# mohammed-amr/detectInBlur

Measured on AMD Instinct MI355X. Metric: blurred imgs/sec @800x1333 (--gpu_blur sparse correlation, fp16, batch 8), higher is better.
Workload: dtype f16; 1 GPU; configs[1]: --gpu_blur batch=8 3x800x1333 fp16, param_index=1 (expl 0.005), low_exposure fractions {1/18,1/10,1/5}, bit-exact accumulation; batch_per_gpu=8, parallelism=image-parallel x1

## Files before the change

### detectinblur_amd/csrc/dib_blur.hip

```cpp
#include "dib_compact_dev.h"
#include <mutex>
#include <stdlib.h>
#include <string.h>

extern "C" { __device__ __attribute__((used)) unsigned *dib_status_word = nullptr; }
#define DIB_STATUS_HANDOFF 1u
#define DIB_STATUS_GEOMETRY 2u
#define DIB_STATUS_WORDS 16
#ifdef DIB_STEP_POLLSTATS
extern "C" { __device__ __attribute__((used)) unsigned dib_poll_stats[4] = {0, 0, 0, 0}; }
#endif

namespace dib {

__device__ __forceinline__ void report_and_exit(unsigned code, unsigned detail) {
  typedef __attribute__((address_space(1))) unsigned gu32;
  gu32 *st = (gu32 *)(size_t)*(unsigned *volatile *)&dib_status_word;
  __hip_atomic_store(st + 1, detail, __ATOMIC_RELAXED, __HIP_MEMORY_SCOPE_SYSTEM);
  __hip_atomic_store(st, code, __ATOMIC_RELAXED, __HIP_MEMORY_SCOPE_SYSTEM);
  __builtin_amdgcn_endpgm();
}

typedef _Float16 h2 __attribute__((ext_vector_type(2)));
typedef unsigned uvec2 __attribute__((ext_vector_type(2)));
// ... 647 lines not shown
      for (int k = 0; k < NK; ++k) {
        bool z;
        coff[k] = 2u * (unsigned)map_coord_sel(c_first + lane + 32 * k, W, pa, pb, mode, z);
        zmask |= z ? 1u << k : 0u;
      }
    }
    if (!zero_mode && r_first >= 0 && r_first + LROWS - 1 <= H - 1) {
      const int s0 = (r_first + qb) * w2;
#pragma unroll
      for (int g = 0; g < GQ; ++g) soff[g] = s0 + g * w2;
    } else {
      const int nrows = TH + (w.rl - w.rf);
#pragma unroll
      for (int g = 0; g < GQ; ++g) {
        bool zr;
        const int sr = map_coord_sel(r_first + min(qb + g, nrows - 1), H, pa, pb, mode, zr);
        zmask |= zr ? 1u << (8 + g) : 0u;
        soff[g] = sr * w2;
      }
    }
    const bool masked = __builtin_amdgcn_ballot_w64(zmask != 0) != 0;
#pragma unroll
    for (int part = 0; part < PARTS; ++part) {
#pragma unroll
      for (int g = 0; g < GP; ++g) {
        if (part * GP + g >= GQ) continue;
        const int so = __builtin_amdgcn_readfirstlane(soff[part * GP + g]);
#pragma unroll
        for (int k = 0; k < NK; ++k) v[g][k] = __builtin_amdgcn_raw_buffer_load_b16(in_rsrc, coff[k], so, 0);
      }
      DIB_TL_STAMP(sg == 0 && part == 0, 40);
      if (part == 0 && sg > 0) __syncthreads();
      const int wl = fresh_lane();
      const unsigned wp = lds0 + (unsigned)((qb + part * GP) * QPITCH + wl * 8);
      if constexpr (L) {
#pragma unroll
        for (int g = 0; g < GP; ++g) {
          if (part * GP + g >= GQ) continue;
          unsigned u[NK];
#pragma unroll
          for (int k = 0; k < NK; ++k)
            u[k] = (masked && (((zmask >> k) & 1u) || ((zmask >> (8 + part * GP + g)) & 1u))) ? 0u : (unsigned)(unsigned short)v[g][k];
          uvec2 e;
          e.x = u[0] | (u[1] << 16);
          e.y = u[2] | (u[3] << 16);
          *(lds_u2 *)(size_t)(wp + (unsigned)(g * QPITCH)) = e;
          if (wl < 32) {
            uvec2 f;
            f.x = u[2] | (u[3] << 16);
            f.y = u[4] | (u[5] << 16);
            *(lds_u2 *)(size_t)(wp + (unsigned)(g * QPITCH + 512)) = f;
          }
        }
      } else if (wl < QUAD_PITCH) {
        if (!masked) {
#pragma unroll
          for (int g = 0; g < GP; ++g) {
            if (part * GP + g >= GQ) continue;
            uvec2 e;
            typedef short s2v __attribute__((ext_vector_type(2)));
            e.x = __builtin_bit_cast(unsigned, s2v{v[g][0], v[g][1]});
            e.y = __builtin_bit_cast(unsigned, s2v{v[g][2], v[g][3]});
            *(lds_u2 *)(size_t)(wp + (unsigned)(g * QPITCH)) = e;
          }
        } else {
#pragma unroll
          for (int g = 0; g < GP; ++g) {
            if (part * GP + g >= GQ) continue;
            unsigned u[4];
#pragma unroll
            for (int k = 0; k < 4; ++k)
              u[k] = (((zmask >> k) & 1u) || ((zmask >> (8 + part * GP + g)) & 1u)) ? 0u : (unsigned)(unsigned short)v[g][k];
            uvec2 e;
            e.x = u[0] | (u[1] << 16);
            e.y = u[2] | (u[3] << 16);
            *(lds_u2 *)(size_t)(wp + (unsigned)(g * QPITCH)) = e;
          }
        }
      }
    }
    __syncthreads();
    DIB_TL_STAMP(sg == 0, 16);
    if constexpr (STEP) { if (sg == 0 && (nsegs >> 30)) wait_tables(); }
    const int tl = fresh_lane();
    const unsigned lane_addr = lds0 + (unsigned)((wave * 8 + (tl >> 5) * 4) * QPITCH + (tl & 31) * 8);
    if constexpr (ACC == DIB_ACC_FP32) {
      if (W - x0f() <= 64) tap_loop_quad_fp32<true, L>(acc32, ltaps, w.t0, w.n, lane_addr);
      else tap_loop_quad_fp32<false, L>(acc32, ltaps, w.t0, w.n, lane_addr);
    } else if constexpr (ACC == DIB_ACC_FAST16) {
      const unsigned long long vg = uniform64((unsigned long long)(tab + table_vgroups_off(K)));
      if (!use_vruns) {
        if (W - x0f() <= 64) tap_loop_quad<true, true, L>(acc, ltaps, w.t0, w.n, lane_addr);
        else tap_loop_quad<true, false, L>(acc, ltaps, w.t0, w.n, lane_addr);
      } else if (W - x0f() <= 64) tap_loop_quad_vrun<true>(acc, vg, w.t0, lane_addr);
      else tap_loop_quad_vrun<false>(acc, vg, w.t0, lane_addr);
    } else {
      if (W - x0f() <= 64) tap_loop_quad<ACC == DIB_ACC_FMA16, true, L>(acc, ltaps, w.t0, w.n, lane_addr);
      else tap_loop_quad<ACC == DIB_ACC_FMA16, false, L>(acc, ltaps, w.t0, w.n, lane_addr);
    }
  }
  if constexpr (ACC == DIB_ACC_FP32) {
#pragma unroll
    for (int i = 0; i < 8; ++i) acc[i] = h2{(_Float16)acc32[2 * i], (_Float16)acc32[2 * i + 1]};
  }
  DIB_TL_STAMP(true, 24);
#undef DIB_TL_STAMP
  if constexpr (NORM) {
    const int Hp = na->Hp, Wp = na->Wp, nhwc = na->nhwc;
    const float m = na->mean[img][ch], sd = na->std[img][ch];
    const unsigned long long a = uniform64((unsigned long long)d.out + (nhwc ? (unsigned long long)ch * 4ull : (unsigned long long)ch * Hp * Wp * 4ull));
    const __amdgpu_buffer_rsrc_t out_rsrc = __builtin_amdgcn_make_buffer_rsrc((void *)a, 0, Hp * Wp * 4 * (nhwc ? 3 : 1) - (nhwc ? ch * 4 : 0), 0x00020000);
    const int x0 = x0f(), y0 = y0f();
    const int sl = fresh_lane();
    const int yl = y0 + wave * 8 + (sl >> 5) * 4, xl = x0 + (sl & 31);
    const unsigned px = nhwc ? 12u : 4u;
    const unsigned base = (unsigned)(yl * Wp + xl) * px, oob = 0x7ffffff0u;
    const bool inside = x0 + QTILE_W <= W && y0 + TH <= H;
#pragma unroll
    for (int i = 0; i < 4; ++i) {
      const unsigned ro = base + (unsigned)(i * Wp) * px;
      const float v[4] = {(float)acc[2 * i].x, (float)acc[2 * i].y, (float)acc[2 * i + 1].x, (float)acc[2 * i + 1].y};
#pragma unroll
      for (int q = 0; q < 4; ++q) {
        const int col = xl + 32 * q, row = yl + i;
        const bool in_img = inside || (row < H && col < W);
        const float f = in_img ? (v[q] - m) / sd : 0.f;
        __builtin_amdgcn_raw_buffer_store_b32(__builtin_bit_cast(int, f), out_rsrc, (in_img || (row < Hp && col < Wp)) ? ro + 32u * q * px : oob, 0, 0);
      }
    }
  } else {
    int chs = ch;
    if constexpr (STEP) asm volatile("" : "+s"(chs));
    const __amdgpu_buffer_rsrc_t out_rsrc = plane_rsrc(d.out, chs, H, W);
    const int x0 = x0f(), y0 = y0f();
    const int sl = fresh_lane();
    const int yl = y0 + wave * 8 + (sl >> 5) * 4, xl = x0 + (sl & 31);
    const unsigned base = (unsigned)(yl * w2 + xl * 2), oob = 0x7ffffff0u;
    if (x0 + QTILE_W <= W && y0 + TH <= H) {
      typedef int i4v __attribute__((ext_vector_type(4)));
      const unsigned long long pa2 = uniform64((unsigned long long)d.out + (unsigned long long)chs * H * W * 2ull);
      const i4v rs = {(int)(unsigned)pa2, (int)(unsigned)(pa2 >> 32) & 0xffff, H * W * 2, 0x00020000};
      int so = 0;
#pragma unroll
      for (int i = 0; i < 4; ++i) {
        asm volatile("buffer_store_short %0, %2, %3, %4 offen\n\t"
                     "buffer_store_short_d16_hi %0, %2, %3, %4 offen offset:64\n\t"
                     "buffer_store_short %1, %2, %3, %4 offen offset:128\n\t"
                     "buffer_store_short_d16_hi %1, %2, %3, %4 offen offset:192"
                     :: "v"(acc[2 * i]), "v"(acc[2 * i + 1]), "v"(base), "s"(rs), "s"(so) : "memory");
        so += w2;
      }
      return;
    }
#pragma unroll
    for (int i = 0; i < 4; ++i) {
      const bool row_ok = yl + i < H;
      const unsigned a0 = __builtin_bit_cast(unsigned, acc[2 * i]), a1 = __builtin_bit_cast(unsigned, acc[2 * i + 1]);
      const unsigned ro = base + (unsigned)(i * w2);
      __builtin_amdgcn_raw_buffer_store_b16((short)(a0 & 0xffffu), out_rsrc, row_ok && xl < W ? ro : oob, 0, 0);
      __builtin_amdgcn_raw_buffer_store_b16((short)(a0 >> 16), out_rsrc, row_ok && xl + 32 < W ? ro + 64u : oob, 0, 0);
      __builtin_amdgcn_raw_buffer_store_b16((short)(a1 & 0xffffu), out_rsrc, row_ok && xl + 64 < W ? ro + 128u : oob, 0, 0);
      __builtin_amdgcn_raw_buffer_store_b16((short)(a1 >> 16), out_rsrc, row_ok && xl + 96 < W ? ro + 192u : oob, 0, 0);
    }
  }
}

#ifdef DIB_TIMELINE
__device__ unsigned long long *g_timeline;
#define DIB_TL_SLOT (*(unsigned long long *volatile *)&g_timeline)
constexpr int TL_WORD = QLDS_BYTES / 4;
#endif

template <int ACC, int KC, bool FLAT = false>
__global__ __launch_bounds__(256, 8) void blur_quad_f16_kernel(BlurBatch batch, FlatBands fb) {
  constexpr int K = KC;
  extern __shared__ unsigned nlds[];
  int img_i = blockIdx.y, entry = blockIdx.x >> 3;
  if constexpr (FLAT) {
    typedef int i16v __attribute__((ext_vector_type(16)));
    const i16v bb = *reinterpret_cast<const i16v *>(fb.begin[blockIdx.x & 7]);
    const int len = bb[15];
// ... 50 lines not shown
  unsigned lds_words;
  __device__ __forceinline__ void operator()() const {
    static_assert(STEP_REPLICA_WORDS * 4 == 128, "the shift below");
#ifdef DIB_PORTABLE_TAPS
    {
      const uvec2 sp = lds_b64(lds_words), tb = lds_b64(lds_words + 8);
      const unsigned xcc = __builtin_amdgcn_s_getreg((2 << 11) | 20);
      const unsigned *ctr = reinterpret_cast<const unsigned *>((((unsigned long long)(unsigned)__builtin_amdgcn_readfirstlane((int)sp.y) << 32) |
                                                                 (unsigned)__builtin_amdgcn_readfirstlane((int)sp.x)) + 128ull * xcc);
      const unsigned target = (unsigned)__builtin_amdgcn_readfirstlane((int)tb.x), budget = (unsigned)__builtin_amdgcn_readfirstlane((int)tb.y);
      for (unsigned spins = 0;; ++spins) {
        if ((int)(__hip_atomic_load(ctr, __ATOMIC_RELAXED, __HIP_MEMORY_SCOPE_AGENT) - target) >= 0) return;
        if (spins >= budget) report_and_exit(DIB_STATUS_HANDOFF, target);
        __builtin_amdgcn_s_sleep(2);
      }
    }
#endif
    asm volatile(
        "v_mov_b32 v48, %0\n\t"
        "ds_read_b64 v[46:47], v48\n\t"
        "ds_read_b64 v[44:45], v48 offset:8\n\t"
        "s_getreg_b32 s39, hwreg(20, 0, 3)\n\t"
        "s_lshl_b32 s39, s39, 7\n\t"
        "s_waitcnt lgkmcnt(0)\n\t"
        "v_readfirstlane_b32 s36, v46\n\t"
        "v_readfirstlane_b32 s37, v47\n\t"
        "v_readfirstlane_b32 s38, v44\n\t"
        "s_add_u32 s36, s36, s39\n\t"
        "s_addc_u32 s37, s37, 0\n\t"
        "v_readfirstlane_b32 s39, v45\n\t"
        "s_load_dword s40, s[36:37], 0x0\n\t"
        "s_mov_b32 s41, 0\n\t"
        "s_waitcnt lgkmcnt(0)\n\t"
        "s_sub_u32 s40, s40, s38\n\t"
        "s_cmp_lt_i32 s40, 0\n\t"
        "s_cbranch_scc0 Ldibw_done%=\n\t"
        "v_mov_b32 v48, 0\n\t"
        "Ldibw_poll%=:\n\t"
        "global_load_dword v48, v48, s[36:37] sc1\n\t"
        "s_waitcnt vmcnt(0)\n\t"
        "v_readfirstlane_b32 s40, v48\n\t"
        "v_mov_b32 v48, 0\n\t"
        "s_sub_u32 s40, s40, s38\n\t"
        "s_cmp_lt_i32 s40, 0\n\t"
        "s_cbranch_scc0 Ldibw_done%=\n\t"
        "s_sleep 2\n\t"
        "s_add_u32 s41, s41, 1\n\t"
        "s_cmp_lt_u32 s41, s39\n\t"
        "s_cbranch_scc1 Ldibw_poll%=\n\t"
        "s_getpc_b64 s[36:37]\n\t"
        "s_add_u32 s36, s36, dib_status_word@rel32@lo+4\n\t"
        "s_addc_u32 s37, s37, dib_status_word@rel32@hi+12\n\t"
        "s_load_dwordx2 s[36:37], s[36:37], 0x0\n\t"
        "v_mov_b32 v47, s38\n\t"
        "v_mov_b32 v46, 1\n\t"
        "s_waitcnt lgkmcnt(0)\n\t"
        "global_store_dword v48, v47, s[36:37] offset:4 sc0 sc1\n\t"
        "global_store_dword v48, v46, s[36:37] sc0 sc1\n\t"
        "s_waitcnt vmcnt(0)\n\t"
        "s_endpgm\n\t"
        "Ldibw_done%=:\n\t"
#ifdef DIB_STEP_POLLSTATS
        "s_cmp_lt_u32 s41, 33\n\t"
        "s_cbranch_scc1 Ldibw_nostat%=\n\t"
        "s_getpc_b64 s[36:37]\n\t"
        "s_add_u32 s36, s36, dib_poll_stats@rel32@lo+4\n\t"
        "s_addc_u32 s37, s37, dib_poll_stats@rel32@hi+12\n\t"
        "v_mov_b32 v48, 0\n\t"
        "global_load_dword v47, v48, s[36:37] offset:4 sc1\n\t"
        "s_waitcnt vmcnt(0)\n\t"
        "v_readfirstlane_b32 s40, v47\n\t"
        "s_cmp_le_u32 s41, s40\n\t"
        "s_cbranch_scc1 Ldibw_nostat%=\n\t"
        "v_mov_b32 v47, s41\n\t"
        "global_atomic_umax v48, v47, s[36:37] offset:4\n\t"
        "Ldibw_nostat%=:\n\t"
#endif
        :: "s"(lds_words)
        : "s36", "s37", "s38", "s39", "s40", "s41", "v44", "v45", "v46", "v47", "v48", "scc", "memory");
  }
};
static_assert(DIB_STATUS_HANDOFF == 1u, "the v_mov_b32 v46, 1 above");

template <int ACC>
__global__ __launch_bounds__(256, 8) void blur_step_f16_kernel(BlurBatch batch, StepSync sy, PsfPtrs psfs) {
  constexpr int K = 128;
  extern __shared__ unsigned nlds[];
  const ImageDesc d = batch.img[blockIdx.y];
  asm volatile("" ::"s"(d.in), "s"(d.out), "s"(d.C), "s"(d.H), "s"(d.W), "s"(d.table), "s"(d.tiles_x), "s"(d.tiles_y),
               "s"(d.inv_per_ch), "s"(d.inv_tiles_x), "s"(d.tab), "s"(sy.sync), "s"(sy.target), "s"(sy.ncx), "s"(sy.row), "s"(sy.rec));
  const int wave = __builtin_amdgcn_readfirstlane((int)threadIdx.x >> 6);
  if (blockIdx.x < (unsigned)sy.ncx) {
    if (blockIdx.y == 0 && blockIdx.x < (unsigned)sy.n_psf && !(sy.flags & COMPACT_DEBUG_NOSIGNAL)) {
      unsigned *rec = sy.rec + (size_t)blockIdx.x * (STEP_REPLICAS * STEP_REC_WORDS);
#ifdef DIB_STEP_STAMPS
      unsigned long long *dbg = *(unsigned long long *volatile *)&g_step_stamps;
      if (dbg) dbg += 8 * blockIdx.x;
      compact_psf_f16_wg256<true, true>(psfs.p[blockIdx.x], sy.flags, sy.tables + (size_t)blockIdx.x * table_words(K), (lds_u32 *)nlds, wave, rec, sy.target, dbg);
#else
      compact_psf_f16_wg256<true, true>(psfs.p[blockIdx.x], sy.flags, sy.tables + (size_t)blockIdx.x * table_words(K), (lds_u32 *)nlds, wave, rec, sy.target);
#endif
      asm volatile("s_waitcnt vmcnt(0)" ::: "memory");
      __syncthreads();
      const int t = wave * 64 + (int)__builtin_amdgcn_mbcnt_hi(~0u, __builtin_amdgcn_mbcnt_lo(~0u, 0u));
#ifdef DIB_STEP_STAMPS
      if (dbg && t == 0) dbg[6] = __builtin_amdgcn_s_memrealtime();
#endif
      if (t < STEP_REPLICAS)
        __hip_atomic_fetch_add(sy.sync + t * STEP_REPLICA_WORDS, 1u, __ATOMIC_RELAXED, __HIP_MEMORY_SCOPE_AGENT);
#ifdef DIB_STEP_STAMPS
      asm volatile("s_waitcnt vmcnt(0)" ::: "memory");
      if (dbg && t == 0) dbg[7] = __builtin_amdgcn_s_memrealtime();
#endif
    }
    return;
  }
  const unsigned bx = blockIdx.x - (unsigned)sy.ncx;
  const int per_ch = d.tiles_x * d.tiles_y;
  int local;
  if (!band_entry(d.C * per_ch, bx & 7, bx >> 3, local)) __builtin_amdgcn_endpgm();
#ifdef DIB_STEP_STAMPS
  unsigned long long *bdbg = *(unsigned long long *volatile *)&g_step_stamps;
  if (bdbg && blockIdx.y == 0 && wave == 0) { bdbg += 8 * MAX_BATCH + 4 * bx; bdbg[0] = __builtin_amdgcn_s_memrealtime(); } else bdbg = nullptr;
#endif
  int early = 1;
  if (blockIdx.y * (unsigned)sy.row + blockIdx.x >= STEP_EARLY) {
    unsigned c;
    asm volatile("s_load_dword %0, %1, 0x0\n\ts_waitcnt lgkmcnt(0)" : "=s"(c) : "s"(sy.sync + (blockIdx.x & 7) * STEP_REPLICA_WORDS) : "memory");
    early = (int)((c - sy.target) >> 31);
  }
  asm volatile("" : "+s"(early));
  int nsegs0 = 0;
  uint4 seg0 = make_uint4(0, 0, 0, 0);
  if (early) {
    const unsigned long long *pr = reinterpret_cast<const unsigned long long *>(sy.rec + ((size_t)d.table * STEP_REPLICAS + (blockIdx.x & (STEP_REPLICAS - 1))) * STEP_REC_WORDS);
#ifdef DIB_STEP_POLLSTATS
    unsigned pspins = 0;
#endif
    for (unsigned spins = 0;; ++spins) {
#ifdef DIB_STEP_POLLSTATS
      pspins = spins;
#endif
      const unsigned long long ra = __hip_atomic_load(pr, __ATOMIC_RELAXED, __HIP_MEMORY_SCOPE_AGENT);
      const unsigned long long rb = __hip_atomic_load(pr + 1, __ATOMIC_RELAXED, __HIP_MEMORY_SCOPE_AGENT);
      const unsigned ta = __builtin_amdgcn_readfirstlane((unsigned)(ra >> 32)), tb = __builtin_amdgcn_readfirstlane((unsigned)(rb >> 32));
      if (ta == sy.target && tb == sy.target) {
        const unsigned a = __builtin_amdgcn_readfirstlane((unsigned)ra), b2 = __builtin_amdgcn_readfirstlane((unsigned)rb);
        nsegs0 = (int)(a >> 16);
        seg0 = make_uint4(0u, a & 0xffffu, b2 >> 16, b2 & 0xffffu);
        break;
      }
      if (spins > sy.poll_budget) report_and_exit(DIB_STATUS_HANDOFF, sy.target);
      __builtin_amdgcn_s_sleep(2);
    }
#ifdef DIB_STEP_POLLSTATS
    if (pspins > 32 && wave == 0 && __builtin_amdgcn_mbcnt_hi(~0u, __builtin_amdgcn_mbcnt_lo(~0u, 0u)) == 0 &&
        pspins > __hip_atomic_load(&dib_poll_stats[0], __ATOMIC_RELAXED, __HIP_MEMORY_SCOPE_AGENT))
      atomicMax(&dib_poll_stats[0], pspins);
#endif
    if (__builtin_amdgcn_mbcnt_hi(~0u, __builtin_amdgcn_mbcnt_lo(~0u, 0u)) == 0) {
      nlds[QLDS_BYTES / 4] = (unsigned)(unsigned long long)sy.sync;
      nlds[QLDS_BYTES / 4 + 1] = (unsigned)((unsigned long long)sy.sync >> 32);
      nlds[QLDS_BYTES / 4 + 2] = sy.target;
      nlds[QLDS_BYTES / 4 + 3] = sy.poll_budget;
    }
    asm volatile("" ::: "memory");
  }
#ifdef DIB_STEP_STAMPS
  if (bdbg) bdbg[1] = __builtin_amdgcn_s_memrealtime();
#endif
  int ch, tx, ty;
  tile_of_local(d, local, ch, tx, ty);
  blur_quad_tile_f16<ACC, false, true>(d, d.tab, K, ch, tx, ty, lds_addr(nlds), wave, early, nsegs0, seg0, StepWait{(unsigned)(size_t)(__attribute__((address_space(3))) char *)nlds + QLDS_BYTES});
#ifdef DIB_STEP_STAMPS
  if (bdbg) { asm volatile("s_waitcnt vmcnt(0)" ::: "memory"); bdbg[2] = __builtin_amdgcn_s_memrealtime(); }
#endif
  __builtin_amdgcn_endpgm();
}

template <int ACC, int KC>
__global__ __launch_bounds__(256, 8) void blur_quad_f16_norm_kernel(BlurBatch batch, NormArgs na) {
  constexpr int K = KC;
  extern __shared__ unsigned nlds[];
  const ImageDesc d = batch.img[blockIdx.y];
  pin_desc(d);
  const int per_ch = d.tiles_x * d.tiles_y;
  int local;
  if (!band_entry(d.C * per_ch, blockIdx.x & 7, blockIdx.x >> 3, local)) return;
  int ch;
  if (na.nhwc) {
    const int t = magic_div(local, 0x55555556u);
    ch = local - 3 * t;
    local = t;
  } else {
    ch = magic_div(local, d.inv_per_ch);
    local -= ch * per_ch;
  }
  const int ty = magic_div(local, d.inv_tiles_x), tx = local - ty * d.tiles_x;
  blur_quad_tile_f16<ACC, false, false, NoWait, true>(d, d.tab, K, ch, tx, ty, lds_addr(nlds), __builtin_amdgcn_readfirstlane((int)threadIdx.x >> 6), 0, 0,
                                                      uint4{0, 0, 0, 0}, NoWait(), &na, (int)blockIdx.y);
}

template <int KC>
__global__ __launch_bounds__(256, 8) void blur_quad_f32acc_kernel(BlurBatch batch) {
  constexpr int K = KC;
  extern __shared__ unsigned nlds[];
  const ImageDesc d = batch.img[blockIdx.y];
  pin_desc(d);
  int ch, tx, ty;
  if (!tile_of_entry(d, blockIdx.x & 7, blockIdx.x >> 3, ch, tx, ty)) return;
  blur_quad_tile_f16<DIB_ACC_FP32>(d, d.tab, K, ch, tx, ty, lds_addr(nlds), __builtin_amdgcn_readfirstlane((int)threadIdx.x >> 6));
}

template <int ACC, int KC>
__global__ __launch_bounds__(256, 4) void blur_quad_large_f16_kernel(BlurBatch batch) {
  constexpr int K = KC;
  extern __shared__ unsigned nlds[];
  const ImageDesc d = batch.img[blockIdx.y];
  int ch, tx, ty;
  if (!tile_of_entry(d, blockIdx.x & 7, blockIdx.x >> 3, ch, tx, ty)) return;
  blur_quad_tile_f16<ACC, true>(d, d.tab, K, ch, tx, ty, lds_addr(nlds), __builtin_amdgcn_readfirstlane((int)threadIdx.x >> 6));
}

template <int ACC>
__global__ __launch_bounds__(64 * NW, NW) void blur_tiled_f16_kernel(BlurBatch batch, const int *__restrict__ tables, int K,
                                                                     unsigned long long *dbg) {
  extern __shared__ uint2 lds[];
  const ImageDesc &d = batch.img[blockIdx.y];
  const int per_ch = d.tiles_x * d.tiles_y;
  int local;
  if (batch.xcd_bands) {
    if (!band_entry(d.C * per_ch, blockIdx.x & 7, blockIdx.x >> 3, local)) return;
// ... 513 lines not shown
```

### detectinblur_amd/csrc/dib_compact_dev.h

```cpp
#pragma once
#include "dib_common.h"
#include <hip/hip_fp16.h>

namespace dib {


__device__ inline long long half_bits_to_fixed(unsigned short h) {
  int sign = h >> 15, e = (h >> 10) & 31, m = h & 1023;
  long long v;
  if (e == 0) v = m;
  else if (e == 31) v = (1ll << 60);
  else v = (long long)(m | 1024) << (e - 1);
  return sign ? -v : v;
}

__device__ inline unsigned short fixed_to_half_bits(long long total) {
  unsigned short sign = total < 0 ? 0x8000 : 0;
  unsigned long long m = total < 0 ? (unsigned long long)(-total) : (unsigned long long)total;
  if (m == 0) return sign;
  int nbits = 64 - __clzll((long long)m);
  if (nbits <= 10) return sign | (unsigned short)m;
  int shift = nbits - 11;
  unsigned long long q = m >> shift, rem = m & ((1ull << shift) - 1);
  if (shift > 0) {
// ... 229 lines not shown
      seg_rlast = seg_r0;
      car_cmin = 1 << 20; car_cmax = -1;
      lo = f;
    }
  }
  if (ntaps > 0) {
    if (lane == 0) {
      st128<WT>(segs + 16 * (size_t)nseg, seg_start, ntaps, (seg_r0 << 8) | seg_rlast, (car_cmin << 8) | car_cmax);
      if (FIRST && nseg == 0) { s_first[0] = seg_start; s_first[1] = ntaps; s_first[2] = (seg_r0 << 8) | seg_rlast; s_first[3] = (car_cmin << 8) | car_cmax; }
    }
    emit_ltaps(seg_start, ntaps, seg_rlast, car_cmax);
    emit_vgroups(seg_start, ntaps, seg_r0, seg_rlast, car_cmin, car_cmax);
    ++nseg;
  } else if (FIRST && lane == 0) {
    s_first[0] = s_first[1] = s_first[2] = s_first[3] = 0;
  }
  if (FIRST && lane == 0) s_first[4] = nseg;
  if (lane < 8) { st32<WT>(ltaps + ntaps + lane, 0u); st32<WT>(ltaps_q + ntaps + lane, 0u); }
  if (lane == 0) st32<WT>(tab + HDR_NSEGS, (unsigned)nseg);
  if constexpr (VG) {
    if (lane == 0) st32<WT>(tab + HDR_K, (unsigned)K | (large ? 1u << 16 : 0u) | ((vg_ok && ntaps > 0) ? HDR_K_VRUNS : 0u));
  }
}

template <bool WT>
__device__ __forceinline__ void segment_positions(int *tab, int K, int flags, int ntaps, const lds_u16 *s_rc, lds_u16 *s_seg,
                                                   lds_u32 *s_sinfo, lds_int *s_first, int lane) {
  char *segs = reinterpret_cast<char *>(tab + table_segs_off(K));
  const bool large = (flags & COMPACT_LARGE_WINDOW) != 0;
  const int seg_rows = large ? SEG_ROWS_L : SEG_ROWS, seg_cols = large ? SEG_COLS_L : SEG_COLS;
  int nseg = 0, seg_start = 0, seg_r0 = 0, seg_rlast = 0, car_cmin = 1 << 20, car_cmax = -1;
  for (int base = 0; base < ntaps; base += 64) {
    const int i = base + lane;
    const bool valid = i < ntaps;
    const unsigned rc = valid ? s_rc[i] : 0u;
    const int r = rc >> 8, c = rc & 255;
    if (base == 0) seg_r0 = __builtin_amdgcn_readlane(r, 0);
    int lo = 0;
    while (true) {
      int pm = wave_scan_min_i32((valid && lane >= lo) ? c : (1 << 20), lane);
      int px = wave_scan_max_i32((valid && lane >= lo) ? c : -1, lane);
      pm = min(pm, car_cmin); px = max(px, car_cmax);
      const bool bad = valid && lane >= lo && ((r - seg_r0 > seg_rows) || (px - pm > seg_cols));
      const unsigned long long fail = __ballot(bad);
      const unsigned long long vmask = __ballot(valid);
      const int last_valid = 63 - __clzll((long long)vmask);
      if (fail == 0) {
        if (valid && lane >= lo) s_seg[i] = (unsigned short)nseg;
        car_cmin = __builtin_amdgcn_readlane(pm, last_valid); car_cmax = __builtin_amdgcn_readlane(px, last_valid);
        seg_rlast = __builtin_amdgcn_readlane(r, last_valid);
        break;
      }
      const int f = __ffsll((long long)fail) - 1;
      if (lane >= lo && lane < f) s_seg[i] = (unsigned short)nseg;
      int cmn = car_cmin, cmx = car_cmax, rl = seg_rlast;
      if (f > lo) { cmn = __builtin_amdgcn_readlane(pm, f - 1); cmx = __builtin_amdgcn_readlane(px, f - 1); rl = __builtin_amdgcn_readlane(r, f - 1); }
      if (lane == 0) {
        st128<WT>(segs + 16 * (size_t)nseg, seg_start, base + f, (seg_r0 << 8) | rl, (cmn << 8) | cmx);
        s_sinfo[nseg] = (unsigned)((rl << 8) | cmx);
        if (nseg == 0) { s_first[0] = seg_start; s_first[1] = base + f; s_first[2] = (seg_r0 << 8) | rl; s_first[3] = (cmn << 8) | cmx; }
      }
      ++nseg;
      seg_start = base + f;
      seg_r0 = __builtin_amdgcn_readlane(r, f);
      seg_rlast = seg_r0;
      car_cmin = 1 << 20; car_cmax = -1;
      lo = f;
    }
  }
  if (ntaps > 0) {
    if (lane == 0) {
      st128<WT>(segs + 16 * (size_t)nseg, seg_start, ntaps, (seg_r0 << 8) | seg_rlast, (car_cmin << 8) | car_cmax);
      s_sinfo[nseg] = (unsigned)((seg_rlast << 8) | car_cmax);
      if (nseg == 0) { s_first[0] = seg_start; s_first[1] = ntaps; s_first[2] = (seg_r0 << 8) | seg_rlast; s_first[3] = (car_cmin << 8) | car_cmax; }
    }
    ++nseg;
  } else if (lane == 0) {
    s_first[0] = s_first[1] = s_first[2] = s_first[3] = 0;
  }
  if (lane == 0) { st32<WT>(tab + HDR_NSEGS, (unsigned)nseg); s_first[4] = nseg; }
}

constexpr int CSTAGE = 1024, CHITS = 512;
template <bool WT, bool EARLY = false>
__device__ __forceinline__ void compact_psf_f16_wg256(const void *psf, int flags, int *tab, lds_u32 *pool, const int wave, unsigned *early = nullptr,
                                                      unsigned tag = 0, unsigned long long *dbg = nullptr) {
#define DIB_CSTAMP(n) do { if (dbg && wave == 0 && lane == 0) dbg[n] = __builtin_amdgcn_s_memrealtime(); } while (0)
  using E = Elem<__half>;
  constexpr int K = 128, LK = 7, NCH = K * K / 8 / 256;
  lds_u16 *s_rc = (lds_u16 *)pool;
  lds_u32 *s_wb = pool + CSTAGE / 2;
  lds_u128 *s_hit = (lds_u128 *)(pool + CSTAGE / 2 + CSTAGE);
  lds_u32 *s_hmeta = pool + CSTAGE / 2 + CSTAGE + 4 * CHITS;
  lds_int *s_tot = (lds_int *)(s_hmeta + CHITS);
  lds_int *s_base = s_tot + NCH * 4;
  lds_i64 *s_part = (lds_i64 *)(s_base + NCH * 4);
  lds_int *s_misc = (lds_int *)(s_part + 4);
  static_assert(((CSTAGE / 2 + CSTAGE) * 4) % 16 == 0 && ((CSTAGE / 2 + CSTAGE + 5 * CHITS + 2 * NCH * 4) * 4) % 8 == 0, "alignment of s_hit / s_part");
  static_assert((CSTAGE / 2 + CSTAGE + 5 * CHITS + 2 * NCH * 4 + 8 + 16) * 4 <= 19712, "fits the blur's window");
  const int lane = (int)__builtin_amdgcn_mbcnt_hi(~0u, __builtin_amdgcn_mbcnt_lo(~0u, 0u));
  const int tid = wave * 64 + lane;
  DIB_CSTAMP(0);
  if (flags & COMPACT_DEBUG_SKIP) {
    if (EARLY && wave == 0 && lane < STEP_REPLICAS) {
      const uint4 s0 = *reinterpret_cast<const uint4 *>(tab + table_segs_off(K));
      st64<true>(early + lane * STEP_REC_WORDS, (s0.y & 0xffffu) | (unsigned)tab[HDR_NSEGS] << 16, tag);
      st64<true>(early + lane * STEP_REC_WORDS + 2, s0.z << 16 | (s0.w & 0xffffu), tag);
    }
    return;
  }
  const uint4 *p4 = reinterpret_cast<const uint4 *>(psf);
  uint4 q[NCH];
#pragma unroll
  for (int i = 0; i < NCH; ++i) q[i] = p4[i * 256 + tid];
  if (tid < 16) s_misc[tid] = (tid < 2 || tid > 5) ? 0 : ((tid & 1) ? -1 : K);
  __syncthreads();
  auto nzmask = [](const uint4 &v) -> unsigned {
    unsigned b = 0;
    b |= (v.x & 0x7fffu) ? 1u : 0u; b |= (v.x & 0x7fff0000u) ? 2u : 0u;
    b |= (v.y & 0x7fffu) ? 4u : 0u; b |= (v.y & 0x7fff0000u) ? 8u : 0u;
    b |= (v.z & 0x7fffu) ? 16u : 0u; b |= (v.z & 0x7fff0000u) ? 32u : 0u;
    b |= (v.w & 0x7fffu) ? 64u : 0u; b |= (v.w & 0x7fff0000u) ? 128u : 0u;
    return b;
  };
  auto half_of = [](const uint4 &v, int k) -> unsigned {
    const unsigned d = (k < 2) ? v.x : (k < 4) ? v.y : (k < 6) ? v.z : v.w;
    return (k & 1) ? d >> 16 : d & 0xffffu;
  };
  const int normalize = flags & COMPACT_NORMALIZE;
  unsigned long long bits = 0;
  {
#pragma unroll
    for (int i = 0; i < NCH; ++i) {
      const unsigned b = ((q[i].x | q[i].y | q[i].z | q[i].w) & 0x7fff7fffu) ? nzmask(q[i]) : 0u;
      bits |= (unsigned long long)b << (8 * i);
      const int c = __popc(b);
      int incl = 0;
      if (__builtin_amdgcn_ballot_w64(b != 0) != 0) {
        incl = wave_scan_incl_i32(c, lane);
        if (b) {
          const int slot = __hip_atomic_fetch_add(&s_misc[6], 1, __ATOMIC_RELAXED, __HIP_MEMORY_SCOPE_WORKGROUP);
          if (slot < CHITS) { s_hit[slot] = lds_vec4{q[i].x, q[i].y, q[i].z, q[i].w}; s_hmeta[slot] = b | (unsigned)(incl - c) << 8 | (unsigned)tid << 18 | (unsigned)i << 26; }
        }
      }
      if (lane == 63) s_tot[i * 4 + wave] = incl;
    }
  }
  DIB_CSTAMP(1);
  __syncthreads();
  int tv = lane < NCH * 4 ? s_tot[lane] : 0;
  int tincl = wave_scan_incl_i32(tv, lane);
  const int n_raw = __builtin_amdgcn_readlane(tincl, NCH * 4 - 1);
  const int nhits = s_misc[6];
  bool ok = n_raw <= CSTAGE && nhits <= CHITS;
  if (ok) {
    if (lane < NCH * 4) s_base[lane] = tincl - tv;
    for (int h = tid; h < nhits; h += 256) {
      const lds_vec4 v = s_hit[h];
      const unsigned m = s_hmeta[h];
      const int i = m >> 26, t = (m >> 18) & 255;
      int pos = s_base[i * 4 + (t >> 6)] + (int)((m >> 8) & 1023);
      const int e0 = (i * 256 + t) * 8;
      const unsigned hw[8] = {v.x & 0xffffu, v.x >> 16, v.y & 0xffffu, v.y >> 16, v.z & 0xffffu, v.z >> 16, v.w & 0xffffu, v.w >> 16};
#pragma unroll
      for (int k = 0; k < 8; ++k)
        if (m & (1u << k)) {
          s_rc[pos] = (unsigned short)((((e0 + k) >> LK) << 8) | ((e0 + k) & (K - 1)));
          s_wb[pos] = hw[k];
          ++pos;
        }
    }
  }
  __syncthreads();
  DIB_CSTAMP(2);
  lds_u16 *s_seg = (lds_u16 *)s_hit;
  lds_u32 *s_sinfo = (lds_u32 *)(s_seg + CSTAGE);
  static_assert(CSTAGE * 2 + CSTAGE * 4 <= CHITS * 16, "segment ids + infos fit the piece list's space");
  __half total = __float2half_rn(1.0f);
  auto publish_first = [&]() {
    if (EARLY && !(flags & COMPACT_NO_SEGMENTS) && lane < STEP_REPLICAS) {
      const unsigned a = (unsigned)s_misc[9] | (unsigned)s_misc[12] << 16;
      const unsigned b = (unsigned)s_misc[10] << 16 | (unsigned)s_misc[11];
      st64<true>(early + lane * STEP_REC_WORDS, a, tag);
      st64<true>(early + lane * STEP_REC_WORDS + 2, b, tag);
    }
  };
  auto row_pointers = [&](int r, int n) {
    const unsigned key = (unsigned)r << 8;
    int lo = 0, hi = n;
    while (lo < hi) { const int mid = (lo + hi) >> 1; if (s_rc[mid] < key) lo = mid + 1; else hi = mid; }
    st32<WT>(tab + table_rowptr_off() + r, (unsigned)lo);
  };
  auto col_extents = [&](int n) {
    int cmn = K, cmx = -1;
    for (int j = lane; j < n; j += 64) { const int c = s_rc[j] & 255; cmn = min(cmn, c); cmx = max(cmx, c); }
    cmn = wave_min_i32(cmn); cmx = wave_max_i32(cmx);
    if (lane == 0) { s_misc[4] = cmn; s_misc[5] = cmx; }
  };
  if (ok) {
    if (wave == 0 && !(flags & COMPACT_NO_SEGMENTS)) segment_positions<WT>(tab, K, flags, n_raw, s_rc, s_seg, s_sinfo, s_misc + 8, lane);
    if (wave == 1) {
      bool lost = false, sane = true;
      if (normalize) {
        long long acc = 0;
        for (int j = lane; j < n_raw; j += 64) acc += E::lift(E::from_bits(s_wb[j]));
        const __half t = E::finish(wave_sum(acc));
        if (lane == 0) s_misc[7] = (int)E::bits(t);
        sane = (float)t == (float)t && E::nonzero(t);
        if (sane)
          for (int j = lane; j < n_raw; j += 64) {
            const __half w = E::div(E::from_bits(s_wb[j]), t);
            lost = lost || !E::nonzero(w);
            s_wb[j] = E::bits(w);
          }
      }
      if (__builtin_amdgcn_ballot_w64(lost) != 0 && lane == 0) s_misc[0] = 1;
      col_extents(n_raw);
    }
    if (wave >= 2) {
      row_pointers((wave - 2) * 64 + lane, n_raw);
      if (wave == 3 && lane == 0) row_pointers(K, n_raw);
    }
  }
  DIB_CSTAMP(3);
  __syncthreads();
  if (ok && normalize) {
    total = E::from_bits((unsigned)s_misc[7]);
    ok = (float)total == (float)total && E::nonzero(total);
  }
  int ntaps = 0;
  if (ok) {
    if (wave == 0 && s_misc[0] == 0) publish_first();
    ntaps = n_raw;
    unsigned *ltaps = reinterpret_cast<unsigned *>(tab + table_ltaps_off(K));
    unsigned *ltaps_q = reinterpret_cast<unsigned *>(tab + table_ltaps_q_off(K));
    if (s_misc[0]) {
      if (wave == 0) {
        int out = 0;
        for (int base = 0; base < n_raw; base += 64) {
          const int j = base + lane;
          const bool valid = j < n_raw;
          const unsigned w = valid ? s_wb[j] : 0u;
          const unsigned short rc = valid ? s_rc[j] : (unsigned short)0;
          const bool keep = valid && (w & 0x7fffu) != 0;
          const unsigned long long km = __builtin_amdgcn_ballot_w64(keep);
          const int pos = out + (int)__builtin_amdgcn_mbcnt_hi((unsigned)(km >> 32), __builtin_amdgcn_mbcnt_lo((unsigned)km, 0));
          if (keep) { s_rc[pos] = rc; s_wb[pos] = w; }
          out += __popcll(km);
        }
        if (lane == 0) s_misc[1] = out;
      }
      __syncthreads();
      ntaps = s_misc[1];
      if (wave == 0 && !(flags & COMPACT_NO_SEGMENTS)) { segment_taps<WT, CSTAGE, true>(tab, K, flags, ntaps, s_rc, s_wb, lane, s_misc + 8); publish_first(); }
      if (wave == 1) col_extents(ntaps);
      if (wave >= 2) {
        row_pointers((wave - 2) * 64 + lane, ntaps);
        if (wave == 3 && lane == 0) row_pointers(K, ntaps);
      }
      __syncthreads();
    } else if (!(flags & COMPACT_NO_SEGMENTS)) {
      const int qpitch = (flags & COMPACT_LARGE_WINDOW) ? QUAD_PITCH_L : QUAD_PITCH;
      for (int j = tid; j < ntaps; j += 256) {
        const unsigned rc = s_rc[j], wj = s_wb[j] & 0xffffu, info = s_sinfo[s_seg[j]];
        const int dr = (int)(info >> 8) - (int)(rc >> 8), dc = (int)(info & 255) - (int)(rc & 255);
        st32<WT>(ltaps + j, (unsigned)((dr * WIN_PITCH + dc) * 8) | (wj << 16));
        st32<WT>(ltaps_q + j, (unsigned)((dr * qpitch + dc) * 8) | (wj << 16));
      }
      if (tid < 8) { st32<WT>(ltaps + ntaps + tid, 0u); st32<WT>(ltaps_q + ntaps + tid, 0u); }
    }
    char *taps = reinterpret_cast<char *>(tab + table_taps_off(K));
    for (int j = tid; j < ntaps; j += 256) st64<WT>(taps + 8 * (size_t)j, (unsigned)s_rc[j], s_wb[j]);
    if (tid == 64) {
      st32<WT>(tab + HDR_NTAPS, (unsigned)ntaps);
      st32<WT>(tab + HDR_RMIN, (unsigned)(ntaps ? (s_rc[0] >> 8) : K)); st32<WT>(tab + HDR_RMAX, (unsigned)(ntaps ? (s_rc[ntaps - 1] >> 8) : -1));
      st32<WT>(tab + HDR_CMIN, (unsigned)s_misc[4]); st32<WT>(tab + HDR_CMAX, (unsigned)s_misc[5]);
      st32<WT>(tab + HDR_K, (unsigned)(K | ((flags & COMPACT_LARGE_WINDOW) ? 1 << 16 : 0))); st32<WT>(tab + HDR_SUM, E::bits(total));
    }
    DIB_CSTAMP(4);
    return;
  } else {
    int nch = NCH, nk = 8;
    asm volatile("" : "+s"(nch), "+s"(nk));
    asm volatile("s_waitcnt vmcnt(0)" ::: "memory");
    __syncthreads();
    if (normalize) {
      long long acc = 0;
  #pragma unroll 1
    for (int i = 0; i < nch; ++i) {
        if (((unsigned)(bits >> (8 * i)) & 0xffu) == 0) continue;
        const uint4 v = p4[i * 256 + tid];
#pragma unroll 1
        for (int k = 0; k < nk; ++k) acc += E::lift(E::from_bits(half_of(v, k)));
      }
      acc = wave_sum(acc);
      __syncthreads();
      if (lane == 0) s_part[wave] = acc;
      __syncthreads();
      const long long part = lane < 4 ? s_part[lane] : 0ll;
      total = E::finish(wave_total(part));
    }
    const bool sane = (float)total == (float)total && E::nonzero(total);
    auto weight = [&](unsigned raw) -> unsigned {
      __half w = E::from_bits(raw);
      if (sane && !E::nonzero(w)) return 0u;
      if (normalize) w = E::div(w, total);
      return E::nonzero(w) ? E::bits(w) : 0u;
    };
    bits = 0;
    int rmin = K, rmax = -1, cmin = K, cmax = -1;
#pragma unroll 1
    for (int i = 0; i < nch; ++i) {
      const uint4 v = p4[i * 256 + tid];
      unsigned b = 0;
      const int e0 = (i * 256 + tid) * 8;
#pragma unroll 1
      for (int k = 0; k < nk; ++k)
        if (weight(half_of(v, k))) {
          b |= 1u << k;
          const int r = (e0 + k) >> LK, c = (e0 + k) & (K - 1);
          rmin = min(rmin, r); rmax = max(rmax, r); cmin = min(cmin, c); cmax = max(cmax, c);
        }
      bits |= (unsigned long long)b << (8 * i);
      const int sc = wave_scan_incl_i32(__popc(b), lane);
      if (lane == 63) s_tot[i * 4 + wave] = sc;
    }
    rmin = wave_min_i32(rmin); rmax = wave_max_i32(rmax); cmin = wave_min_i32(cmin); cmax = wave_max_i32(cmax);
    if (lane == 0) {
      __hip_atomic_fetch_min(&s_misc[2], rmin, __ATOMIC_RELAXED, __HIP_MEMORY_SCOPE_WORKGROUP); __hip_atomic_fetch_max(&s_misc[3], rmax, __ATOMIC_RELAXED, __HIP_MEMORY_SCOPE_WORKGROUP);
      __hip_atomic_fetch_min(&s_misc[4], cmin, __ATOMIC_RELAXED, __HIP_MEMORY_SCOPE_WORKGROUP); __hip_atomic_fetch_max(&s_misc[5], cmax, __ATOMIC_RELAXED, __HIP_MEMORY_SCOPE_WORKGROUP);
    }
    __syncthreads();
    tv = lane < NCH * 4 ? s_tot[lane] : 0;
    tincl = wave_scan_incl_i32(tv, lane);
    ntaps = __builtin_amdgcn_readlane(tincl, NCH * 4 - 1);
    char *taps = reinterpret_cast<char *>(tab + table_taps_off(K));
#pragma unroll 1
    for (int i = 0; i < nch; ++i) {
      const int base = __builtin_amdgcn_readlane(tincl - tv, i * 4 + wave);
      const unsigned b = (unsigned)(bits >> (8 * i)) & 0xffu;
      const int cb = __popc(b);
      int pos = base + wave_scan_incl_i32(cb, lane) - cb;
      const int e0 = (i * 256 + tid) * 8;
      if ((tid & 15) == 0) st32<WT>(tab + table_rowptr_off() + 16 * i + (tid >> 4), (unsigned)pos);
      if (b == 0) continue;
      const uint4 v = p4[i * 256 + tid];
#pragma unroll 1
      for (int k = 0; k < nk; ++k)
        if (b & (1u << k)) {
          const unsigned rc = (unsigned)((((e0 + k) >> LK) << 8) | ((e0 + k) & (K - 1))), wb = weight(half_of(v, k));
          st64<WT>(taps + 8 * (size_t)pos, rc, wb);
          if (pos < CSTAGE) { s_rc[pos] = (unsigned short)rc; s_wb[pos] = wb; }
          ++pos;
        }
    }
    if (tid == 0) {
      st32<WT>(tab + table_rowptr_off() + K, (unsigned)ntaps);
      st32<WT>(tab + HDR_NTAPS, (unsigned)ntaps);
      st32<WT>(tab + HDR_RMIN, (unsigned)s_misc[2]); st32<WT>(tab + HDR_RMAX, (unsigned)s_misc[3]);
      st32<WT>(tab + HDR_CMIN, (unsigned)s_misc[4]); st32<WT>(tab + HDR_CMAX, (unsigned)s_misc[5]);
      st32<WT>(tab + HDR_K, (unsigned)(K | ((flags & COMPACT_LARGE_WINDOW) ? 1 << 16 : 0))); st32<WT>(tab + HDR_SUM, E::bits(total));
    }
    asm volatile("s_waitcnt vmcnt(0)" ::: "memory");
    __threadfence_block();
    __syncthreads();
  }
  if (wave == 0 && !(flags & COMPACT_NO_SEGMENTS)) { segment_taps<WT, CSTAGE, true>(tab, K, flags, ntaps, s_rc, s_wb, lane, s_misc + 8); publish_first(); }
#undef DIB_CSTAMP
}

}
```

Before: 184,400 images/s.

## Publish early PSF bounding box and signal blur blocks before full table write

The PSF compaction blocks now record the nonzero bounding box in an extra early handoff record once the taps are found to fit one segment. Blur blocks that are polling can pick up this box and begin with a provisional single-segment window, rebasing their LDS address once the real segment header arrives. The step signal is moved inside the compaction routine so it fires after the quad tap table and headers are written, deferring the non-quad ltaps and raw tap writes until after the signal. This shortens the critical handoff between table building and convolution, at the cost of added atomics, a more complex protocol, and a risk of ordering bugs.

```diff
diff --git a/detectinblur_amd/csrc/dib_blur.hip b/detectinblur_amd/csrc/dib_blur.hip
--- a/detectinblur_amd/csrc/dib_blur.hip
+++ b/detectinblur_amd/csrc/dib_blur.hip
@@ -753,21 +753,35 @@
     __syncthreads();
     DIB_TL_STAMP(sg == 0, 16);
     if constexpr (STEP) { if (sg == 0 && (nsegs >> 30)) wait_tables(); }
+    int t0 = w.t0, n = w.n;
+    unsigned rebase = 0;
+    if constexpr (STEP) {
+      if (sg == 0 && ((nsegs >> 29) & 1)) {
+        unsigned __int128 r;
+        unsigned ns;
+        asm volatile("s_load_dword %0, %2, 0x1c\n\ts_load_dwordx4 %1, %3, 0x0\n\ts_waitcnt lgkmcnt(0)"
+                     : "=&s"(ns), "=&s"(r) : "s"((unsigned long long)tab), "s"((unsigned long long)segs) : "memory");
+        if (ns == 0) break;
+        const int raw = n;
+        t0 = (int)(unsigned)r; n = (int)(unsigned)(r >> 32) - t0;
+        rebase = (unsigned)((((raw >> 8) - (int)((unsigned)(r >> 64) & 255u)) * QUAD_PITCH + ((raw & 255) - (int)((unsigned)(r >> 96) & 255u))) * 8);
+      }
+    }
     const int tl = fresh_lane();
-    const unsigned lane_addr = lds0 + (unsigned)((wave * 8 + (tl >> 5) * 4) * QPITCH + (tl & 31) * 8);
+    const unsigned lane_addr = lds0 + (unsigned)((wave * 8 + (tl >> 5) * 4) * QPITCH + (tl & 31) * 8) + rebase;
     if constexpr (ACC == DIB_ACC_FP32) {
-      if (W - x0f() <= 64) tap_loop_quad_fp32<true, L>(acc32, ltaps, w.t0, w.n, lane_addr);
-      else tap_loop_quad_fp32<false, L>(acc32, ltaps, w.t0, w.n, lane_addr);
+      if (W - x0f() <= 64) tap_loop_quad_fp32<true, L>(acc32, ltaps, t0, n, lane_addr);
+      else tap_loop_quad_fp32<false, L>(acc32, ltaps, t0, n, lane_addr);
     } else if constexpr (ACC == DIB_ACC_FAST16) {
       const unsigned long long vg = uniform64((unsigned long long)(tab + table_vgroups_off(K)));
       if (!use_vruns) {
-        if (W - x0f() <= 64) tap_loop_quad<true, true, L>(acc, ltaps, w.t0, w.n, lane_addr);
-        else tap_loop_quad<true, false, L>(acc, ltaps, w.t0, w.n, lane_addr);
-      } else if (W - x0f() <= 64) tap_loop_quad_vrun<true>(acc, vg, w.t0, lane_addr);
-      else tap_loop_quad_vrun<false>(acc, vg, w.t0, lane_addr);
+        if (W - x0f() <= 64) tap_loop_quad<true, true, L>(acc, ltaps, t0, n, lane_addr);
+        else tap_loop_quad<true, false, L>(acc, ltaps, t0, n, lane_addr);
+      } else if (W - x0f() <= 64) tap_loop_quad_vrun<true>(acc, vg, t0, lane_addr);
+      else tap_loop_quad_vrun<false>(acc, vg, t0, lane_addr);
     } else {
-      if (W - x0f() <= 64) tap_loop_quad<ACC == DIB_ACC_FMA16, true, L>(acc, ltaps, w.t0, w.n, lane_addr);
-      else tap_loop_quad<ACC == DIB_ACC_FMA16, false, L>(acc, ltaps, w.t0, w.n, lane_addr);
+      if (W - x0f() <= 64) tap_loop_quad<ACC == DIB_ACC_FMA16, true, L>(acc, ltaps, t0, n, lane_addr);
+      else tap_loop_quad<ACC == DIB_ACC_FMA16, false, L>(acc, ltaps, t0, n, lane_addr);
     }
   }
   if constexpr (ACC == DIB_ACC_FP32) {
@@ -984,6 +998,27 @@
 };
 static_assert(DIB_STATUS_HANDOFF == 1u, "the v_mov_b32 v46, 1 above");
 
+struct StepSignal {
+  static constexpr bool active = true;
+  unsigned *sync;
+  int wave;
+  unsigned long long *dbg;
+  __device__ __forceinline__ void operator()() const {
+    asm volatile("s_waitcnt vmcnt(0)" ::: "memory");
+    __syncthreads();
+    const int t = wave * 64 + (int)__builtin_amdgcn_mbcnt_hi(~0u, __builtin_amdgcn_mbcnt_lo(~0u, 0u));
+#ifdef DIB_STEP_STAMPS
+    if (dbg && t == 0) dbg[6] = __builtin_amdgcn_s_memrealtime();
+#endif
+    if (t < STEP_REPLICAS)
+      __hip_atomic_fetch_add((__attribute__((address_space(1))) unsigned *)(size_t)(sync + t * STEP_REPLICA_WORDS), 1u, __ATOMIC_RELAXED, __HIP_MEMORY_SCOPE_AGENT);
+#ifdef DIB_STEP_STAMPS
+    asm volatile("s_waitcnt vmcnt(0)" ::: "memory");
+    if (dbg && t == 0) dbg[7] = __builtin_amdgcn_s_memrealtime();
+#endif
+  }
+};
+
 template <int ACC>
 __global__ __launch_bounds__(256, 8) void blur_step_f16_kernel(BlurBatch batch, StepSync sy, PsfPtrs psfs) {
   constexpr int K = 128;
@@ -995,24 +1030,17 @@
   if (blockIdx.x < (unsigned)sy.ncx) {
     if (blockIdx.y == 0 && blockIdx.x < (unsigned)sy.n_psf && !(sy.flags & COMPACT_DEBUG_NOSIGNAL)) {
       unsigned *rec = sy.rec + (size_t)blockIdx.x * (STEP_REPLICAS * STEP_REC_WORDS);
+      unsigned long long *dbg = nullptr;
 #ifdef DIB_STEP_STAMPS
-      unsigned long long *dbg = *(unsigned long long *volatile *)&g_step_stamps;
+      dbg = *(unsigned long long *volatile *)&g_step_stamps;
       if (dbg) dbg += 8 * blockIdx.x;
+#endif
+      const StepSignal sig{sy.sync, wave, dbg};
+#if DIB_STEP_VARIANT & 2
+      compact_psf_f16_wg256<true, true, StepSignal>(psfs.p[blockIdx.x], sy.flags, sy.tables + (size_t)blockIdx.x * table_words(K), (lds_u32 *)nlds, wave, rec, sy.target, dbg, sig);
+#else
       compact_psf_f16_wg256<true, true>(psfs.p[blockIdx.x], sy.flags, sy.tables + (size_t)blockIdx.x * table_words(K), (lds_u32 *)nlds, wave, rec, sy.target, dbg);
-#else
-      compact_psf_f16_wg256<true, true>(psfs.p[blockIdx.x], sy.flags, sy.tables + (size_t)blockIdx.x * table_words(K), (lds_u32 *)nlds, wave, rec, sy.target);
-#endif
-      asm volatile("s_waitcnt vmcnt(0)" ::: "memory");
-      __syncthreads();
-      const int t = wave * 64 + (int)__builtin_amdgcn_mbcnt_hi(~0u, __builtin_amdgcn_mbcnt_lo(~0u, 0u));
-#ifdef DIB_STEP_STAMPS
-      if (dbg && t == 0) dbg[6] = __builtin_amdgcn_s_memrealtime();
-#endif
-      if (t < STEP_REPLICAS)
-        __hip_atomic_fetch_add(sy.sync + t * STEP_REPLICA_WORDS, 1u, __ATOMIC_RELAXED, __HIP_MEMORY_SCOPE_AGENT);
-#ifdef DIB_STEP_STAMPS
-      asm volatile("s_waitcnt vmcnt(0)" ::: "memory");
-      if (dbg && t == 0) dbg[7] = __builtin_amdgcn_s_memrealtime();
+      sig();
 #endif
     }
     return;
@@ -1045,11 +1073,18 @@
 #endif
       const unsigned long long ra = __hip_atomic_load(pr, __ATOMIC_RELAXED, __HIP_MEMORY_SCOPE_AGENT);
       const unsigned long long rb = __hip_atomic_load(pr + 1, __ATOMIC_RELAXED, __HIP_MEMORY_SCOPE_AGENT);
+      const unsigned long long rp = __hip_atomic_load(pr + 2, __ATOMIC_RELAXED, __HIP_MEMORY_SCOPE_AGENT);
       const unsigned ta = __builtin_amdgcn_readfirstlane((unsigned)(ra >> 32)), tb = __builtin_amdgcn_readfirstlane((unsigned)(rb >> 32));
       if (ta == sy.target && tb == sy.target) {
         const unsigned a = __builtin_amdgcn_readfirstlane((unsigned)ra), b2 = __builtin_amdgcn_readfirstlane((unsigned)rb);
         nsegs0 = (int)(a >> 16);
         seg0 = make_uint4(0u, a & 0xffffu, b2 >> 16, b2 & 0xffffu);
+        break;
+      }
+      if (__builtin_amdgcn_readfirstlane((unsigned)(rp >> 32)) == sy.target) {
+        const unsigned box = __builtin_amdgcn_readfirstlane((unsigned)rp);
+        nsegs0 = 1 | 1 << 29;
+        seg0 = make_uint4(0u, (box >> 8 & 0xff00u) | (box & 0xffu), box >> 16, box & 0xffffu);
         break;
       }
       if (spins > sy.poll_budget) report_and_exit(DIB_STATUS_HANDOFF, sy.target);
diff --git a/detectinblur_amd/csrc/dib_compact_dev.h b/detectinblur_amd/csrc/dib_compact_dev.h
--- a/detectinblur_amd/csrc/dib_compact_dev.h
+++ b/detectinblur_amd/csrc/dib_compact_dev.h
@@ -335,9 +335,13 @@
 }
 
 constexpr int CSTAGE = 1024, CHITS = 512;
-template <bool WT, bool EARLY = false>
+#ifndef DIB_STEP_VARIANT
+#define DIB_STEP_VARIANT 3
+#endif
+struct NoSignal { static constexpr bool active = false; __device__ void operator()() const {} };
+template <bool WT, bool EARLY = false, typename Sig = NoSignal>
 __device__ __forceinline__ void compact_psf_f16_wg256(const void *psf, int flags, int *tab, lds_u32 *pool, const int wave, unsigned *early = nullptr,
-                                                      unsigned tag = 0, unsigned long long *dbg = nullptr) {
+                                                      unsigned tag = 0, unsigned long long *dbg = nullptr, const Sig sig = Sig()) {
 #define DIB_CSTAMP(n) do { if (dbg && wave == 0 && lane == 0) dbg[n] = __builtin_amdgcn_s_memrealtime(); } while (0)
   using E = Elem<__half>;
   constexpr int K = 128, LK = 7, NCH = K * K / 8 / 256;
@@ -350,7 +354,7 @@
   lds_i64 *s_part = (lds_i64 *)(s_base + NCH * 4);
   lds_int *s_misc = (lds_int *)(s_part + 4);
   static_assert(((CSTAGE / 2 + CSTAGE) * 4) % 16 == 0 && ((CSTAGE / 2 + CSTAGE + 5 * CHITS + 2 * NCH * 4) * 4) % 8 == 0, "alignment of s_hit / s_part");
-  static_assert((CSTAGE / 2 + CSTAGE + 5 * CHITS + 2 * NCH * 4 + 8 + 16) * 4 <= 19712, "fits the blur's window");
+  static_assert((CSTAGE / 2 + CSTAGE + 5 * CHITS + 2 * NCH * 4 + 8 + 24) * 4 <= 19712, "fits the blur's window");
   const int lane = (int)__builtin_amdgcn_mbcnt_hi(~0u, __builtin_amdgcn_mbcnt_lo(~0u, 0u));
   const int tid = wave * 64 + lane;
   DIB_CSTAMP(0);
@@ -360,6 +364,7 @@
       st64<true>(early + lane * STEP_REC_WORDS, (s0.y & 0xffffu) | (unsigned)tab[HDR_NSEGS] << 16, tag);
       st64<true>(early + lane * STEP_REC_WORDS + 2, s0.z << 16 | (s0.w & 0xffffu), tag);
     }
+    sig();
     return;
   }
   const uint4 *p4 = reinterpret_cast<const uint4 *>(psf);
@@ -367,6 +372,7 @@
 #pragma unroll
   for (int i = 0; i < NCH; ++i) q[i] = p4[i * 256 + tid];
   if (tid < 16) s_misc[tid] = (tid < 2 || tid > 5) ? 0 : ((tid & 1) ? -1 : K);
+  if (EARLY && tid >= 16 && tid < 24) s_misc[tid] = tid > 19 ? 0 : ((tid & 1) ? -1 : K);
   __syncthreads();
   auto nzmask = [](const uint4 &v) -> unsigned {
     unsigned b = 0;
@@ -382,6 +388,9 @@
   };
   const int normalize = flags & COMPACT_NORMALIZE;
   unsigned long long bits = 0;
+  auto odd_pair = [](unsigned x) -> unsigned {
+    return (((x & 0x7fffu) != 0 && (x & 0xffffu) >= 0x7c00u) || ((x & 0x7fff0000u) != 0 && x >= 0x7c000000u)) ? 1u : 0u;
+  };
   {
 #pragma unroll
     for (int i = 0; i < NCH; ++i) {
@@ -394,6 +403,13 @@
         if (b) {
           const int slot = __hip_atomic_fetch_add(&s_misc[6], 1, __ATOMIC_RELAXED, __HIP_MEMORY_SCOPE_WORKGROUP);
           if (slot < CHITS) { s_hit[slot] = lds_vec4{q[i].x, q[i].y, q[i].z, q[i].w}; s_hmeta[slot] = b | (unsigned)(incl - c) << 8 | (unsigned)tid << 18 | (unsigned)i << 26; }
+          if constexpr (EARLY) {
+            const int r = i * 16 + (tid >> 4), c0 = (tid & 15) * 8;
+            __hip_atomic_fetch_min(&s_misc[16], r, __ATOMIC_RELAXED, __HIP_MEMORY_SCOPE_WORKGROUP); __hip_atomic_fetch_max(&s_misc[17], r, __ATOMIC_RELAXED, __HIP_MEMORY_SCOPE_WORKGROUP);
+            __hip_atomic_fetch_min(&s_misc[18], c0 + __builtin_ctz(b), __ATOMIC_RELAXED, __HIP_MEMORY_SCOPE_WORKGROUP);
+            __hip_atomic_fetch_max(&s_misc[19], c0 + 31 - __builtin_clz(b), __ATOMIC_RELAXED, __HIP_MEMORY_SCOPE_WORKGROUP);
+            if (odd_pair(q[i].x) | odd_pair(q[i].y) | odd_pair(q[i].z) | odd_pair(q[i].w)) __hip_atomic_fetch_or(&s_misc[20], 1, __ATOMIC_RELAXED, __HIP_MEMORY_SCOPE_WORKGROUP);
+          }
         }
       }
       if (lane == 63) s_tot[i * 4 + wave] = incl;
@@ -406,6 +422,12 @@
   const int n_raw = __builtin_amdgcn_readlane(tincl, NCH * 4 - 1);
   const int nhits = s_misc[6];
   bool ok = n_raw <= CSTAGE && nhits <= CHITS;
+  if (EARLY && (DIB_STEP_VARIANT & 1) && wave == 0 && ok && n_raw > 0 && normalize && !(flags & (COMPACT_NO_SEGMENTS | COMPACT_LARGE_WINDOW))) {
+    const int r0 = s_misc[16], r1 = s_misc[17], c0 = s_misc[18], c1 = s_misc[19];
+    if (r1 - r0 <= SEG_ROWS && c1 - c0 <= SEG_COLS && s_misc[20] == 0 && lane < STEP_REPLICAS)
+      st64<true>(early + lane * STEP_REC_WORDS + 4, (unsigned)((r0 << 8 | r1) << 16 | c0 << 8 | c1), tag);
+    DIB_CSTAMP(5);
+  }
   if (ok) {
     if (lane < NCH * 4) s_base[lane] = tincl - tv;
     for (int h = tid; h < nhits; h += 256) {
@@ -487,6 +509,7 @@
     ntaps = n_raw;
     unsigned *ltaps = reinterpret_cast<unsigned *>(tab + table_ltaps_off(K));
     unsigned *ltaps_q = reinterpret_cast<unsigned *>(tab + table_ltaps_q_off(K));
+    char *taps = reinterpret_cast<char *>(tab + table_taps_off(K));
     if (s_misc[0]) {
       if (wave == 0) {
         int out = 0;
@@ -517,18 +540,31 @@
       for (int j = tid; j < ntaps; j += 256) {
         const unsigned rc = s_rc[j], wj = s_wb[j] & 0xffffu, info = s_sinfo[s_seg[j]];
         const int dr = (int)(info >> 8) - (int)(rc >> 8), dc = (int)(info & 255) - (int)(rc & 255);
-        st32<WT>(ltaps + j, (unsigned)((dr * WIN_PITCH + dc) * 8) | (wj << 16));
+        if constexpr (!Sig::active) st32<WT>(ltaps + j, (unsigned)((dr * WIN_PITCH + dc) * 8) | (wj << 16));
         st32<WT>(ltaps_q + j, (unsigned)((dr * qpitch + dc) * 8) | (wj << 16));
       }
-      if (tid < 8) { st32<WT>(ltaps + ntaps + tid, 0u); st32<WT>(ltaps_q + ntaps + tid, 0u); }
-    }
-    char *taps = reinterpret_cast<char *>(tab + table_taps_off(K));
+      if (tid < 8) { if constexpr (!Sig::active) st32<WT>(ltaps + ntaps + tid, 0u); st32<WT>(ltaps_q + ntaps + tid, 0u); }
+    }
+    if (tid == 64) {
+      st32<WT>(tab + HDR_CMAX, (unsigned)s_misc[5]);
+      st32<WT>(tab + HDR_K, (unsigned)(K | ((flags & COMPACT_LARGE_WINDOW) ? 1 << 16 : 0))); st32<WT>(tab + HDR_SUM, E::bits(total));
+    }
+    if constexpr (Sig::active) {
+      sig();
+      if (s_misc[0] == 0 && !(flags & COMPACT_NO_SEGMENTS)) {
+        for (int j = tid; j < ntaps; j += 256) {
+          const unsigned rc = s_rc[j], wj = s_wb[j] & 0xffffu, info = s_sinfo[s_seg[j]];
+          const int dr = (int)(info >> 8) - (int)(rc >> 8), dc = (int)(info & 255) - (int)(rc & 255);
+          st32<WT>(ltaps + j, (unsigned)((dr * WIN_PITCH + dc) * 8) | (wj << 16));
+        }
+        if (tid < 8) st32<WT>(ltaps + ntaps + tid, 0u);
+      }
+    }
     for (int j = tid; j < ntaps; j += 256) st64<WT>(taps + 8 * (size_t)j, (unsigned)s_rc[j], s_wb[j]);
     if (tid == 64) {
       st32<WT>(tab + HDR_NTAPS, (unsigned)ntaps);
       st32<WT>(tab + HDR_RMIN, (unsigned)(ntaps ? (s_rc[0] >> 8) : K)); st32<WT>(tab + HDR_RMAX, (unsigned)(ntaps ? (s_rc[ntaps - 1] >> 8) : -1));
-      st32<WT>(tab + HDR_CMIN, (unsigned)s_misc[4]); st32<WT>(tab + HDR_CMAX, (unsigned)s_misc[5]);
-      st32<WT>(tab + HDR_K, (unsigned)(K | ((flags & COMPACT_LARGE_WINDOW) ? 1 << 16 : 0))); st32<WT>(tab + HDR_SUM, E::bits(total));
+      st32<WT>(tab + HDR_CMIN, (unsigned)s_misc[4]);
     }
     DIB_CSTAMP(4);
     return;
@@ -619,6 +655,7 @@
     __syncthreads();
   }
   if (wave == 0 && !(flags & COMPACT_NO_SEGMENTS)) { segment_taps<WT, CSTAGE, true>(tab, K, flags, ntaps, s_rc, s_wb, lane, s_misc + 8); publish_first(); }
+  sig();
 #undef DIB_CSTAMP
 }
 
```

New measurement: 171,400 images/s. 7.1% lower.
